# keyber/Single-Image-Super-Resolution

Measured on AMD Instinct MI355X. Metric: HR patches/sec (x2 generator fwd+bwd, LR 96x96 -> SR 192x192), higher is better.
Workload: dtype f32; 1 GPU; SRGAN x2 generator (16 blocks, 64 features, spectral norm) fwd+bwd+Adam with bicubic LR degradation and pixel-MSE x10, per-GPU batch 16 HR 192x192 patches (LR 96x96 -> SR 192x192): the north star's headline. BASELINE.json's metric string "96^2 crops, x4" is configs.cfg3 of this line. Single build: fp32.; per_gpu_batch=16, hr=192, lr=96, parallelism=dp1, hip_graph=True

## Files before the change

single-image-super-resolution_amd/csrc/conv_trunk_f32.hip:

```cpp
#include "sisr_dev.h"
#include "sisr_bf16_stage.h"
#include "sisr_instr.h"

typedef unsigned cf_u32x4 __attribute__((ext_vector_type(4)));

#include <algorithm>
#include <cstdlib>
#include <type_traits>

#define CF_TH 8
#define CF_TW 16
#define CF_IH (CF_TH + 2)
#define CF_IW (CF_TW + 2)
#define CF_NPIX (CF_IH * CF_IW)
#define CF_PSF 36
#define CF_HALO_BYTES (CF_NPIX * CF_PSF * 4)
#define CF_WROW 36
#define CF_WCHUNK_BYTES (9 * 32 * CF_WROW * 4)
#define CF_ITEMS ((CF_NPIX * 8 + 255) / 256)
#define CF_THREADS 512
#define CF_KROWP 100
#define CF_PS 33

SISR_TRACE_BUFFER(sisr_cftrace, 512, 128)
#define CFT(k) SISR_TRACE_STAMP(sisr_cftrace, threadIdx.x == 0, blockIdx.x, k, 64, wall_clock64())
#define CFTP(k) SISR_TRACE_STAMP(sisr_cftrace, threadIdx.x == 256, blockIdx.x, 64 + (k), 128, wall_clock64())
SISR_TRACE_BUFFER(sisr_cfclk, 512, 2)
#define CFTC(k) SISR_TRACE_STAMP(sisr_cfclk, threadIdx.x == 0, blockIdx.x, (k) - 60, 2, clock64())

struct CTrunkF32Args {
    const float *x1, *x2;
    float* x_out;
    BnFinArgs fin;
    const float *pa, *pb, *pd, *ps, *pt;
    const float* slope_p; float slope;
    const float* wpk;
    const void* wimg;
    const float* bias;
    const float* res;
    float* y;
    float *stat_part, *cnt_part;
    const float *bnb_x, *bnb_scale, *bnb_shift, *bnb_mean, *bnb_invstd, *bnb_slope_p;
    float bnb_slope; int bnb_act;
    float* bnb_part;
    int N, H, W;
    int tiles_x, per_img, total, streams;
    uint32_t m_tiles_x, m_per_img;
    int glog, cout_pad, shuffle;
    int xsc, xph;
};

__device__ __forceinline__ __amdgpu_buffer_rsrc_t cf_rsrc(const void* p, unsigned bytes) {
    return __builtin_amdgcn_make_buffer_rsrc(const_cast<void*>(p), 0, (int)bytes, 0x00020000);
}

__device__ __forceinline__ void cf_split2(float v0, float v1, unsigned& hw, unsigned& lw) {
    const f32x2 v = {v0, v1};
    hw = __builtin_bit_cast(unsigned, __builtin_convertvector(v, bf16x2));
    const f32x2 r = {v0 - __uint_as_float(hw << 16), v1 - __uint_as_float(hw & 0xFFFF0000u)};
    lw = __builtin_bit_cast(unsigned, __builtin_convertvector(r, bf16x2));
}

template <int PRO, bool SPLIT>
__global__ void __launch_bounds__(CF_THREADS, 2) conv_trunk_f32_kernel(const CTrunkF32Args a) {
    extern __shared__ __attribute__((aligned(16))) unsigned char lds[];
    unsigned char* halo0 = lds + 2 * CF_WCHUNK_BYTES;
    float* red = reinterpret_cast<float*>(halo0 + 2 * CF_HALO_BYTES);

    const int tid = threadIdx.x, lane = tid & 63;
    const int wave = __builtin_amdgcn_readfirstlane(tid >> 6);
    const bool consumer = wave < 4;
    const int l31 = lane & 31, kk = lane >> 5;
    const bool xcd = (a.streams & 7) == 0;
    const int hc = xcd ? (blockIdx.x >> 3) & ((1 << a.glog) - 1) : blockIdx.x & ((1 << a.glog) - 1);
    const int stream = xcd ? (blockIdx.x & 7) | ((blockIdx.x >> (3 + a.glog)) << 3) : blockIdx.x >> a.glog;
    const unsigned tbytes = (unsigned)a.N * (unsigned)a.H * (unsigned)a.W * 256u;
    constexpr bool TWO = PRO == SISR_PRO_BNBWD || PRO == SISR_PRO_BNACT_BWD || PRO == SISR_PRO_RES_AFFINE || PRO == SISR_PRO_ACT_BWD;
    constexpr bool SUM = PRO == SISR_PRO_RES_AFFINE;
    auto tile_coords = [&](int T, int& n, int& ty, int& tx) {
        n = fdiv(T, a.m_per_img);
        const int rem = T - n * a.per_img;
        ty = fdiv(rem, a.m_tiles_x);
        tx = rem - ty * a.tiles_x;
    };

    CFT(0);
    CFTC(60);
    float* kfin = red + 4 * 32 * 3;
    const bool fin = (PRO == SISR_PRO_AFFINE_ACT || PRO == SISR_PRO_RES_AFFINE) && a.fin.stat != nullptr;
    if (fin) bn_finalize_in_kernel(a.fin, reinterpret_cast<double*>(lds), kfin, blockIdx.x == 0);
    auto fill_weights = [&]() {
        float* wl = reinterpret_cast<float*>(lds);
        if (a.wimg != nullptr) {
            constexpr int UNITS = 2 * 9 * 32 * CF_WROW / 4;
            constexpr int W_IT16 = (UNITS + CF_THREADS - 1) / CF_THREADS;
            const cf_u32x4* src = reinterpret_cast<const cf_u32x4*>(a.wimg) + hc * UNITS;
            cf_u32x4 wv16[W_IT16];
#pragma unroll
            for (int it = 0; it < W_IT16; ++it) {
                const int u = tid + it * CF_THREADS;
                wv16[it] = u < UNITS ? src[u] : cf_u32x4{0u, 0u, 0u, 0u};
            }
#pragma unroll
            for (int it = 0; it < W_IT16; ++it) {
                const int u = tid + it * CF_THREADS;
                if (u < UNITS) reinterpret_cast<cf_u32x4*>(wl)[u] = wv16[it];
            }
            return;
        }
        constexpr int W_IT = 2 * 9 * 32 * 32 / CF_THREADS;
        float wv[W_IT];
#pragma unroll
        for (int it = 0; it < W_IT; ++it) {
            const int e = tid + it * CF_THREADS;
            const int ci = e & 31, s = (e >> 5) % 3, t2 = (e >> 5) / 3;
            const int co = t2 & 31, qr = t2 >> 5;
            wv[it] = a.wpk[((int64_t)qr * a.cout_pad + 32 * hc + co) * CF_KROWP + s * CF_PS + ci];
        }
#pragma unroll
        for (int it = 0; it < W_IT; ++it) {
            const int e = tid + it * CF_THREADS;
            const int ci = e & 31, s = (e >> 5) % 3, t2 = (e >> 5) / 3;
            const int co = t2 & 31, qr = t2 >> 5;
            const int q = qr / 3, r = qr - 3 * q;
            if constexpr (SPLIT) {
                const float vo = __shfl_xor(wv[it], 1);
                const bool odd = ci & 1;
                unsigned hw, lw;
                cf_split2(odd ? vo : wv[it], odd ? wv[it] : vo, hw, lw);
                reinterpret_cast<unsigned*>(wl)[((q * 9 + r * 3 + s) * 32 + co) * CF_WROW + (odd ? 16 : 0) + (ci >> 1)] = odd ? lw : hw;
            } else {
                wl[((q * 9 + r * 3 + s) * 32 + co) * CF_WROW + ci] = wv[it];
            }
        }
    };

    const int n_mine = stream < a.total ? (a.total - stream + a.streams - 1) / a.streams : 0;
    const int n_stages = 2 * n_mine;

    if (!consumer) {
        const int pt = tid & 255, quad = tid & 7, m0 = pt >> 3;
        const int tiles_y = a.per_img / a.tiles_x;
        const float slope = PRO != SISR_PRO_NONE ? (a.slope_p ? a.slope_p[0] : a.slope) : 1.f;
        f32x4 ka[2], kb[2], kd[2], ks[2], kt[2];
        int rel[CF_ITEMS];
        unsigned flags = 0;
#pragma unroll
        for (int k = 0; k < CF_ITEMS; ++k) {
            const int px = m0 + 32 * k;
            const int py = px / CF_IW, pxx = px - py * CF_IW;
            rel[k] = ((py - 1) * a.xsc * a.xsc * a.W + (pxx - 1) * a.xsc) * 256 + quad * 16;
            const unsigned f = (py == 0 ? 1u : 0u) | (py == CF_IH - 1 ? 2u : 0u) | (pxx == 0 ? 4u : 0u) | (pxx == CF_IW - 1 ? 8u : 0u) |
                               (px >= CF_NPIX ? 16u : 0u);
            flags |= f << (5 * k);
            asm volatile("" : "+v"(rel[k]));
        }
        const bool last_beyond = m0 + 32 * (CF_ITEMS - 1) >= CF_NPIX;
        const int ldso = SPLIT ? m0 * CF_PSF * 4 + quad * 8 : (m0 * CF_PSF + quad * 4) * 4;
        const bool easy_slope = slope >= 0.f && slope <= 1.f;

        struct Stage { f32x4 s1[CF_ITEMS], s2[CF_ITEMS]; unsigned bad, origin; bool edge; };
        Stage stA, stB;
        auto issue = [&](int j, Stage& st) {
            const int T = stream + (j >> 1) * a.streams, q = j & 1;
            const unsigned xbytes = (unsigned)(a.xsc * a.xsc) * tbytes;
            const __amdgpu_buffer_rsrc_t r1 = cf_rsrc(a.x1, xbytes), r2 = cf_rsrc(TWO ? a.x2 : a.x1, xbytes);
            int n, ty, tx;
            tile_coords(T, n, ty, tx);
            const unsigned origin = (unsigned)(((n * a.xsc * a.H + a.xsc * ty * CF_TH + (a.xph >> 1)) * a.xsc * a.W + a.xsc * tx * CF_TW + (a.xph & 1)) * 256 + q * 128);
            const unsigned e = (ty == 0 ? 1u : 0u) | (ty == tiles_y - 1 ? 2u : 0u) | (tx == 0 ? 4u : 0u) | (tx == a.tiles_x - 1 ? 8u : 0u);
            st.edge = e != 0u;
            st.bad = flags & ((e | 16u) * 0x02108421u);
            st.origin = origin;
#pragma unroll
            for (int k = 0; k < CF_ITEMS; ++k) {
                const unsigned voff = origin + (unsigned)rel[k];
                st.s1[k] = __builtin_bit_cast(f32x4, __builtin_amdgcn_raw_buffer_load_b128(r1, voff, 0, 0));
                if (TWO) st.s2[k] = __builtin_bit_cast(f32x4, __builtin_amdgcn_raw_buffer_load_b128(r2, voff, 0, 0));
            }
        };
        auto commit_t = [&](auto easy_, auto edge_, int j, const Stage& st) {
            constexpr int EASY = decltype(easy_)::value;
            constexpr bool EDGE = decltype(edge_)::value;
            const int q = j & 1;
            float* img = reinterpret_cast<float*>(halo0 + (j & 1) * CF_HALO_BYTES + ldso);
            const f32x4 qa = q ? ka[1] : ka[0], qb = q ? kb[1] : kb[0], qd = q ? kd[1] : kd[0], qs = q ? ks[1] : ks[0], qt = q ? kt[1] : kt[0];
            const __amdgpu_buffer_rsrc_t ro = cf_rsrc(SUM ? a.x_out : a.x1, tbytes);
#pragma unroll
            for (int k = 0; k < CF_ITEMS; ++k) {
                if (k == CF_ITEMS - 1 && last_beyond) break;
                const bool ok = !EDGE || ((st.bad >> (5 * k)) & 31u) == 0u;
                auto value = [&](int c) {
                    const float v = st.s1[k][c];
                    if (PRO == SISR_PRO_NONE) return v;
                    if (PRO == SISR_PRO_ACT) return lrelu_t<EASY>(v, slope);
                    if (PRO == SISR_PRO_AFFINE_ACT) return lrelu_t<EASY>(qa[c] * v + qd[c], slope);
                    if (SUM) return lrelu_t<EASY>(v, slope) + (qa[c] * st.s2[k][c] + qd[c]);
                    if (PRO == SISR_PRO_ACT_BWD) return st.s2[k][c] > 0.f ? v : slope * v;
                    const float bx = st.s2[k][c];
                    float g = v;
                    if (PRO == SISR_PRO_BNACT_BWD) g = qs[c] * bx + qt[c] > 0.f ? v : slope * v;
                    return qa[c] * g + qb[c] * bx + qd[c];
                };
                const f32x4 osum = {value(0), value(1), value(2), value(3)};
                const f32x4 zero4 = {0.f, 0.f, 0.f, 0.f};
                if constexpr (SPLIT) {
                    typedef unsigned cf_u32x2 __attribute__((ext_vector_type(2)));
                    unsigned h0, l0, h1, l1;
                    cf_split2(osum[0], osum[1], h0, l0);
                    cf_split2(osum[2], osum[3], h1, l1);
                    const cf_u32x2 hw = {h0, h1}, lw = {l0, l1};
                    const cf_u32x2 z2 = {0u, 0u};
                    *reinterpret_cast<cf_u32x2*>(img + k * 32 * CF_PSF) = ok ? hw : z2;
                    *reinterpret_cast<cf_u32x2*>(img + k * 32 * CF_PSF + 16) = ok ? lw : z2;
                } else
                *reinterpret_cast<f32x4*>(img + k * 32 * CF_PSF) = ok ? osum : zero4;
                if (SUM && hc == 0 && ((flags >> (5 * k)) & 31u) == 0u)
                    __builtin_amdgcn_raw_buffer_store_b128(__builtin_bit_cast(cf_u32x4, osum), ro, st.origin + (unsigned)rel[k], 0, 0);
            }
        };
        auto commit = [&](int j, const Stage& st) {
            using T1 = std::integral_constant<int, 1>; using T0 = std::integral_constant<int, 0>;
            constexpr bool HAS_ACT = PRO == SISR_PRO_ACT || PRO == SISR_PRO_AFFINE_ACT || SUM;
            if (!HAS_ACT || easy_slope) {
                if (st.edge) commit_t(T1{}, std::true_type{}, j, st); else commit_t(T1{}, std::false_type{}, j, st);
            } else {
                if (st.edge) commit_t(T0{}, std::true_type{}, j, st); else commit_t(T0{}, std::false_type{}, j, st);
            }
        };

        issue(0, stA);
        issue(1, stB);
#pragma unroll
        for (int q = 0; q < 2; ++q)
#pragma unroll
            for (int j = 0; j < 4; ++j) {
                const int c = q * 32 + quad * 4 + j;
                constexpr bool AFF = PRO == SISR_PRO_AFFINE_ACT || (TWO && PRO != SISR_PRO_ACT_BWD);
                ka[q][j] = fin ? kfin[c] : AFF ? a.pa[c] : 1.f;
                kd[q][j] = fin ? kfin[64 + c] : AFF ? a.pd[c] : 0.f;
                kb[q][j] = (TWO && !SUM && PRO != SISR_PRO_ACT_BWD) ? a.pb[c] : 0.f;
                ks[q][j] = PRO == SISR_PRO_BNACT_BWD ? a.ps[c] : 0.f;
                kt[q][j] = PRO == SISR_PRO_BNACT_BWD ? a.pt[c] : 0.f;
            }
        fill_weights();
        __syncthreads();
        if (n_stages > 0) commit(0, stA);
        __syncthreads();
        int j = 0;
        while (j < n_stages) {
            CFTP(4 + 6 * j);
            issue(j + 2, stA);
            CFTP(5 + 6 * j);
            if (j + 1 < n_stages) commit(j + 1, stB);
            CFTP(8 + 6 * j);
            __syncthreads();
            CFTP(9 + 6 * j);
            if (++j >= n_stages) break;
            CFTP(4 + 6 * j);
            issue(j + 2, stB);
            CFTP(5 + 6 * j);
            if (j + 1 < n_stages) commit(j + 1, stA);
            CFTP(8 + 6 * j);
            __syncthreads();
            CFTP(9 + 6 * j);
            ++j;
        }
    } else {
        const int co = a.shuffle ? 32 * (hc & 1) + l31 : 32 * hc + l31;
        const int ph = hc >> 1;
        const int abase = SPLIT ? ((2 * wave + (l31 >> 4)) * CF_IW + (l31 & 15)) * CF_PSF * 4 + 16 * kk
                                : (((2 * wave + (l31 >> 4)) * CF_IW + (l31 & 15)) * CF_PSF + 16 * kk) * 4;
        const int bbase = SPLIT ? l31 * CF_WROW * 4 + 16 * kk : (l31 * CF_WROW + 16 * kk) * 4;
        const float bv = a.bias != nullptr ? a.bias[a.shuffle ? co * 4 + ph : co] : 0.f;
        float st_shift = 0.f, st_s1 = 0.f, st_s2 = 0.f;
        int st_n = 0;
        const __amdgpu_buffer_rsrc_t ry = cf_rsrc(a.y, a.shuffle ? 4u * tbytes : tbytes), rr = cf_rsrc(a.res != nullptr ? a.res : a.y, tbytes);
        f32x16 acc;
        f32x16 rv, xv;
        const bool has_x = a.bnb_part != nullptr;
        const __amdgpu_buffer_rsrc_t rxb = cf_rsrc(has_x ? a.bnb_x : a.y, tbytes);
        float b_sc = 0.f, b_sf = 0.f, b_mu = 0.f, b_is = 0.f, b_slope = 1.f;
        float rs1 = 0.f, rs2 = 0.f, rsl = 0.f;
        if (has_x) {
            b_sc = a.bnb_scale[co]; b_sf = a.bnb_shift[co]; b_mu = a.bnb_mean[co]; b_is = a.bnb_invstd[co];
            b_slope = a.bnb_slope_p ? a.bnb_slope_p[0] : a.bnb_slope;
        }
        fill_weights();
        __syncthreads();
        __syncthreads();
        for (int j = 0; j < n_stages; ++j) {
            const int q = j & 1;
            CFT(4 + 6 * j);
            int n, ty, tx;
            tile_coords(stream + (j >> 1) * a.streams, n, ty, tx);
            const unsigned obase = a.shuffle ? (unsigned)((((n * 2 * a.H + 2 * (ty * CF_TH + 2 * wave) + (ph >> 1)) * 2 * a.W + 2 * tx * CF_TW + (ph & 1)) * 64 + co) * 4)
                                             : (unsigned)((((n * a.H + ty * CF_TH + 2 * wave) * a.W + tx * CF_TW) * 64 + co) * 4);
            const int orow = a.shuffle ? 4 * a.W * 256 : a.W * 256, ocol = a.shuffle ? 512 : 256;
            if (q == 0) {
#pragma unroll
                for (int i = 0; i < 16; ++i) acc[i] = bv;
            } else {
                if (a.res != nullptr) {
#pragma unroll
                    for (int i = 0; i < 16; ++i) {
                        const int p = mfma_row(i, lane);
                        rv[i] = __builtin_bit_cast(float, __builtin_amdgcn_raw_buffer_load_b32(rr, obase + (unsigned)(((p >> 4) * a.W + (p & 15)) * 256), 0, 0));
                    }
                }
                if (has_x) {
#pragma unroll
                    for (int i = 0; i < 16; ++i) {
                        const int p = mfma_row(i, lane);
                        xv[i] = __builtin_bit_cast(float, __builtin_amdgcn_raw_buffer_load_b32(rxb, obase + (unsigned)(((p >> 4) * a.W + (p & 15)) * 256), 0, 0));
                    }
                }
            }
            const unsigned char* ab = halo0 + (j & 1) * CF_HALO_BYTES + abase;
            const unsigned char* bb = lds + q * CF_WCHUNK_BYTES + bbase;
            if constexpr (SPLIT) {
                bf16x8 ah[9][2], al[9][2], bh[9][2], bl[9][2];
                auto fetch_s = [&](int t) {
                    const unsigned char* pa = ab + ((t / 3) * CF_IW + (t % 3)) * CF_PSF * 4;
                    const unsigned char* pb = bb + t * 32 * CF_WROW * 4;
#pragma unroll
                    for (int ks = 0; ks < 2; ++ks) {
                        ah[t][ks] = *reinterpret_cast<const bf16x8*>(pa + 32 * ks);
                        bh[t][ks] = *reinterpret_cast<const bf16x8*>(pb + 32 * ks);
                        al[t][ks] = *reinterpret_cast<const bf16x8*>(pa + 64 + 32 * ks);
                        bl[t][ks] = *reinterpret_cast<const bf16x8*>(pb + 64 + 32 * ks);
                    }
                };
                fetch_s(0);
                fetch_s(1);
                __builtin_amdgcn_sched_barrier(0);
#pragma unroll
                for (int t = 0; t < 9; ++t) {
                    if (t + 2 < 9) fetch_s(t + 2);
#pragma unroll
                    for (int ks = 0; ks < 2; ++ks) {
                        acc = __builtin_amdgcn_mfma_f32_32x32x16_bf16(al[t][ks], bh[t][ks], acc, 0, 0, 0);
                        acc = __builtin_amdgcn_mfma_f32_32x32x16_bf16(ah[t][ks], bl[t][ks], acc, 0, 0, 0);
                        acc = __builtin_amdgcn_mfma_f32_32x32x16_bf16(ah[t][ks], bh[t][ks], acc, 0, 0, 0);
                    }
                    __builtin_amdgcn_sched_barrier(0);
                }
            } else {
            f32x4 af[18][2], bf[18][2];
            auto fetch = [&](int u) {
                const int t = u >> 1, s0 = 8 * (u & 1);
#pragma unroll
                for (int v = 0; v < 2; ++v) {
                    af[u][v] = *reinterpret_cast<const f32x4*>(ab + (((t / 3) * CF_IW + (t % 3)) * CF_PSF + s0 + 4 * v) * 4);
                    bf[u][v] = *reinterpret_cast<const f32x4*>(bb + ((t * 32) * CF_WROW + s0 + 4 * v) * 4);
                }
            };
            fetch(0);
            fetch(1);
            __builtin_amdgcn_sched_group_barrier(0x100, 8, 0);
#pragma unroll
            for (int u = 0; u < 18; ++u) {
                if (u + 2 < 18) fetch(u + 2);
#pragma unroll
                for (int s = 0; s < 8; ++s) acc = __builtin_amdgcn_mfma_f32_32x32x2f32(af[u][s >> 2][s & 3], bf[u][s >> 2][s & 3], acc, 0, 0, 0);
                if (u + 2 < 18) __builtin_amdgcn_sched_group_barrier(0x100, 4, 0);
                __builtin_amdgcn_sched_group_barrier(0x008, 8, 0);
            }
            }
            CFT(6 + 6 * j);
            if (q == 1) {
                if (a.res != nullptr) {
#pragma unroll
                    for (int i = 0; i < 16; ++i) acc[i] += rv[i];
                }
                if (has_x) {
                    if (a.bnb_act) {
#pragma unroll
                        for (int i = 0; i < 16; ++i) {
                            float gv = acc[i];
                            const float z = b_sc * xv[i] + b_sf;
                            const bool neg = !(z > 0.f);
                            rsl += neg ? gv * z : 0.f;
                            gv = neg ? gv * b_slope : gv;
                            rs1 += gv;
                            rs2 += gv * ((xv[i] - b_mu) * b_is);
                        }
                    } else {
#pragma unroll
                        for (int i = 0; i < 16; ++i) {
                            rs1 += acc[i];
                            rs2 += acc[i] * ((xv[i] - b_mu) * b_is);
                        }
                    }
                }
                if (a.stat_part != nullptr) {
                    if (st_n == 0) {
                        float s = 0.f;
#pragma unroll
                        for (int i = 0; i < 16; ++i) s += acc[i];
                        st_shift = s * (1.f / 16.f);
                    }
#pragma unroll
                    for (int i = 0; i < 16; ++i) {
                        const float dv = acc[i] - st_shift;
                        st_s1 += dv;
                        st_s2 += dv * dv;
                    }
                    st_n += 16;
                }
#pragma unroll
                for (int i = 0; i < 16; ++i) {
                    const int p = mfma_row(i, lane);
                    __builtin_amdgcn_raw_buffer_store_b32(__builtin_bit_cast(unsigned, (float)acc[i]), ry,
                                                          obase + (unsigned)((p >> 4) * orow + (p & 15) * ocol), 0, 0);
                }
            }
            CFT(8 + 6 * j);
            __syncthreads();
            CFT(9 + 6 * j);
        }
        CFT(3);

        if (a.stat_part != nullptr) {
            float nn = (float)st_n, mu = 0.f, m2 = 0.f;
            if (st_n > 0) {
                const float m1 = st_s1 / nn;
                mu = st_shift + m1;
                m2 = st_s2 - st_s1 * m1;
            }
            const float nb = __shfl_xor(nn, 32), mub = __shfl_xor(mu, 32), m2b = __shfl_xor(m2, 32);
            const float nt = nn + nb;
            if (nt > 0.f) { const float dl = mub - mu, f = nb / nt; mu += dl * f; m2 += m2b + dl * dl * nn * f; }
            nn = nt;
            if (kk == 0) { float* r = red + (wave * 32 + l31) * 3; r[0] = nn; r[1] = mu; r[2] = m2; }
        }
        if (has_x) {
            rs1 += __shfl_xor(rs1, 32);
            rs2 += __shfl_xor(rs2, 32);
            rsl += __shfl_xor(rsl, 32);
            if (kk == 0) { float* r = red + (wave * 32 + l31) * 3; r[0] = rs1; r[1] = rs2; r[2] = rsl; }
        }
    }
    if (a.bnb_part != nullptr) {
        __syncthreads();
        float* wk = a.bnb_part + (int64_t)blockIdx.x * 129;
        if (tid < 64) {
            const int c = tid & 31;
            const bool mine = (tid >> 5) == hc;
            float s1 = 0.f, s2 = 0.f;
            if (mine) {
                s1 = (red[c * 3] + red[(32 + c) * 3]) + (red[(64 + c) * 3] + red[(96 + c) * 3]);
                s2 = (red[c * 3 + 1] + red[(32 + c) * 3 + 1]) + (red[(64 + c) * 3 + 1] + red[(96 + c) * 3 + 1]);
            }
            wk[tid] = s1;
            wk[64 + tid] = s2;
        }
        if (tid == 64) {
            float sl = 0.f;
            for (int i = 0; i < 128; ++i) sl += red[i * 3 + 2];
            wk[128] = sl;
        }
    }
    if (a.stat_part != nullptr) {
        __syncthreads();
        if (tid < 32) {
            float nn = red[tid * 3], mm = red[tid * 3 + 1], qq = red[tid * 3 + 2];
#pragma unroll
            for (int w = 1; w < 4; ++w) {
                const float* r1 = red + (w * 32 + tid) * 3;
                const float nb = r1[0], nt = nn + nb;
                if (nt > 0.f) { const float dl = r1[1] - mm, f = nb / nt; mm += dl * f; qq += r1[2] + dl * dl * nn * f; }
                nn = nt;
            }
            float* sp = a.stat_part + (int64_t)stream * 128 + 32 * hc + tid;
            sp[0] = mm;
            sp[64] = qq;
            if (tid == 0 && hc == 0) a.cnt_part[stream] = nn;
        }
    }
    CFT(63);
    CFTC(61);
}

static int cf_streams(const SisrConvDesc* d) {
    const int total = d->N * (d->H / CF_TH) * (d->W / CF_TW);
    const int cus = sisr_cu_slots();
    const int slots = std::max(1, cus / (d->Cout == 256 ? 8 : 2));
    const int rounds = (total + slots - 1) / slots;
    return (total + rounds - 1) / rounds;
}

extern "C" int sisr_conv2d_trunk_f32_eligible(const SisrConvDesc* d) {
    if (!d || sisr_switch_off("SISR_TRUNK")) return 0;
    if (sisr_switch_off("SISR_TRUNK_F32CONV")) return 0;
    const bool up_off = sisr_switch_off("SISR_TRUNK_UP");
    if (!up_off && d->Cin == 256 && d->Cout == 64 && d->KH == 3 && d->KW == 3 && d->stride == 1 && d->pad_y == 1 && d->pad_x == 1 &&
        d->x_mode == SISR_X_NHWC_UNSHUFFLE2 && d->pro_mode == SISR_PRO_ACT_BWD && d->x2 && d->y_mode == SISR_Y_NHWC && !d->x_bf16 && !d->y_bf16 &&
        !d->res_bf16 && d->Ho == d->H && d->Wo == d->W && !(d->H % CF_TH) && !(d->W % CF_TW) && d->y_sy == 1 && d->y_sx == 1 && !d->y_oy && !d->y_ox &&
        d->y_H == d->Ho && d->y_W == d->Wo && d->epi_act == SISR_EPI_NONE && d->plan.CK == 32 && d->plan.PS == CF_PS && d->plan.KROWP == CF_KROWP &&
        d->plan.CoutPad == 64 && d->plan.n_chunk == 8 && (int64_t)d->N * d->H * d->W * 1024 < (1ll << 31) &&
        d->N * (d->H / CF_TH) * (d->W / CF_TW) < 65536 && !d->stat_part && !d->bias && !d->bnb_part && !d->fin_stat)
        return 2;
    if (d->Cin != 64 || d->KH != 3 || d->KW != 3 || d->stride != 1 || d->pad_y != 1 || d->pad_x != 1) return 0;
    const bool up = !up_off && d->Cout == 256 && d->y_mode == SISR_Y_NHWC_SHUFFLE2 && d->plan.CoutPad == 256 && !d->stat_part &&
                    !d->res && !d->bnb_part && !d->fin_stat &&
                    (d->pro_mode == SISR_PRO_NONE || d->pro_mode == SISR_PRO_ACT || d->pro_mode == SISR_PRO_AFFINE_ACT);
    if (!up && (d->Cout != 64 || d->y_mode != SISR_Y_NHWC || d->plan.CoutPad != 64)) return 0;
    if (d->x_mode != SISR_X_NHWC || d->x_bf16 || d->y_bf16 || d->res_bf16) return 0;
    if (d->Ho != d->H || d->Wo != d->W || (d->H % CF_TH) || (d->W % CF_TW)) return 0;
    if (!up && (d->y_sy != 1 || d->y_sx != 1 || d->y_oy || d->y_ox || d->y_H != d->Ho || d->y_W != d->Wo)) return 0;
    if (d->epi_act != SISR_EPI_NONE) return 0;
    if (d->plan.CK != 32 || d->plan.PS != CF_PS || d->plan.KROWP != CF_KROWP || d->plan.n_chunk != 2) return 0;
    if ((int64_t)d->N * d->H * d->W * 256 * (up ? 4 : 1) >= (1ll << 31)) return 0;
    if (d->N * (d->H / CF_TH) * (d->W / CF_TW) >= 65536) return 0;
    const bool fwd_pro = d->pro_mode == SISR_PRO_NONE || d->pro_mode == SISR_PRO_ACT || d->pro_mode == SISR_PRO_AFFINE_ACT ||
                         (d->pro_mode == SISR_PRO_RES_AFFINE && d->x2 && d->x_out && ((d->pa && d->pd) || d->fin_stat));
    if (d->fin_stat && !((d->pro_mode == SISR_PRO_AFFINE_ACT || d->pro_mode == SISR_PRO_RES_AFFINE) && d->fin_cnt && d->fin_gamma &&
                         d->fin_beta && d->fin_rm && d->fin_rv && d->fin_k && d->fin_rows > 0))
        return 0;
    if (fwd_pro && !d->res && !d->bnb_part) return 1;
    const bool bwd_pro = d->pro_mode == SISR_PRO_BNBWD || d->pro_mode == SISR_PRO_BNACT_BWD;
    if (bwd_pro && !d->stat_part && !d->bias && (!d->bnb_part || (d->bnb_x && !d->bnbx_bf16))) return 2;
    return 0;
}

extern "C" int sisr_conv2d_f32_parts(const SisrConvDesc* d) {
    if (!d) return SISR_E_BADARG;
    return sisr_conv2d_trunk_f32_eligible(d) ? cf_streams(d) : d->plan.n_tiles;
}

extern "C" int sisr_conv2d_f32_bnb_parts(const SisrConvDesc* d) {
    if (!d) return SISR_E_BADARG;
    return sisr_conv2d_trunk_f32_eligible(d) == 2 ? 2 * cf_streams(d) : 0;
}

template <int PRO, bool SPLIT>
static int launch_cf_t(const CTrunkF32Args& a, hipStream_t st) {
    constexpr int lds_bytes = 2 * CF_WCHUNK_BYTES + 2 * CF_HALO_BYTES + 4 * 32 * 3 * 4 + 128 * 4;
    return sisr_launch<conv_trunk_f32_kernel<PRO, SPLIT>>(dim3(a.streams << a.glog), dim3(CF_THREADS), lds_bytes, 0, st, a);
}
template <int PRO>
static int launch_cf(const CTrunkF32Args& a, bool split, hipStream_t st) {
    return split ? launch_cf_t<PRO, true>(a, st) : launch_cf_t<PRO, false>(a, st);
}

int sisr_conv2d_trunk_f32_launch(const SisrConvDesc* d, hipStream_t st) {
    if (operand_needs_x2(d->pro_mode) && !d->x2) return SISR_E_BADARG;
    CTrunkF32Args a{};
    a.fin.stat = d->fin_stat; a.fin.cnt = d->fin_cnt; a.fin.gamma = d->fin_gamma; a.fin.beta = d->fin_beta;
    a.fin.rm = d->fin_rm; a.fin.rv = d->fin_rv; a.fin.k = d->fin_k; a.fin.rows = d->fin_rows; a.fin.momentum = d->fin_momentum; a.fin.eps = d->fin_eps;
    a.x1 = d->x1; a.x2 = d->x2; a.x_out = d->x_out; a.pa = d->pa; a.pb = d->pb; a.pd = d->pd; a.ps = d->ps; a.pt = d->pt;
    a.slope_p = d->pro_slope_p; a.slope = d->pro_slope;
    a.wpk = d->wpk; a.bias = d->bias; a.res = d->res; a.y = d->y; a.stat_part = d->stat_part; a.cnt_part = d->cnt_part;
    const int img_mode = (d->plan.variant >> 1) & 3;
    a.wimg = (d->Cin == 64 && d->Cout == 64 && img_mode == (d->mfma_split ? 2 : 1)) ? static_cast<const void*>(d->wpk + d->plan.wpk_elems) : nullptr;
    a.N = d->N; a.H = d->H; a.W = d->W;
    a.tiles_x = d->W / CF_TW; a.per_img = (d->H / CF_TH) * a.tiles_x; a.total = d->N * a.per_img;
    a.streams = cf_streams(d);
    a.glog = d->Cout == 256 ? 3 : 1; a.cout_pad = d->Cout == 256 ? 256 : 64; a.shuffle = d->y_mode == SISR_Y_NHWC_SHUFFLE2 ? 1 : 0;
    a.bnb_x = d->bnb_x; a.bnb_scale = d->bnb_scale; a.bnb_shift = d->bnb_shift; a.bnb_mean = d->bnb_mean; a.bnb_invstd = d->bnb_invstd;
    a.bnb_slope_p = d->bnb_slope_p; a.bnb_slope = d->bnb_slope; a.bnb_act = d->bnb_act; a.bnb_part = d->bnb_part;
    a.m_tiles_x = fdiv_magic(a.tiles_x); a.m_per_img = fdiv_magic(a.per_img);
    a.xsc = 1; a.xph = 0;
    if (d->Cin == 256) {
        a.xsc = 2;
        for (int ph = 0; ph < 4; ++ph) {
            a.xph = ph;
            a.wpk = d->wpk + (size_t)ph * 2 * 3 * 64 * CF_KROWP;
            a.res = ph == 0 ? d->res : d->y;
            if (int e = launch_cf<SISR_PRO_ACT_BWD>(a, d->mfma_split != 0, st)) return e;
        }
        return 0;
    }
    switch (d->pro_mode) {
        case SISR_PRO_NONE: return launch_cf<SISR_PRO_NONE>(a, d->mfma_split != 0, st);
        case SISR_PRO_ACT: return launch_cf<SISR_PRO_ACT>(a, d->mfma_split != 0, st);
        case SISR_PRO_AFFINE_ACT: return launch_cf<SISR_PRO_AFFINE_ACT>(a, d->mfma_split != 0, st);
        case SISR_PRO_BNBWD: return launch_cf<SISR_PRO_BNBWD>(a, d->mfma_split != 0, st);
        case SISR_PRO_BNACT_BWD: return launch_cf<SISR_PRO_BNACT_BWD>(a, d->mfma_split != 0, st);
        case SISR_PRO_RES_AFFINE: return launch_cf<SISR_PRO_RES_AFFINE>(a, d->mfma_split != 0, st);
    }
    return SISR_E_UNSUPPORTED;
}
```

Baseline: 1453 HR patches/s.

## Widen trunk conv tiles to 48 columns with swizzled 16-channel halo stages

Adds a template group count G so each tile covers 16*G columns (G=3 when W is a multiple of 48 and the wave-quantization check passes), giving each consumer wave G accumulators that reuse the same weight fragments. The halo is restaged in four 16-channel slices with an XOR-swizzled pixel layout instead of two 32-channel padded rows, and the per-channel affine constants move from producer registers into an LDS table. The intent is to amortize weight LDS reads and per-tile overhead over more output pixels and cut bank conflicts. The cost is more LDS per block, more registers per consumer, and fewer tiles, which can hurt load balance across CUs.

After: 1452 HR patches/s. Within noise of the previous version (-0.1%).

```diff
diff --git a/single-image-super-resolution_amd/csrc/conv_trunk_f32.hip b/single-image-super-resolution_amd/csrc/conv_trunk_f32.hip
--- a/single-image-super-resolution_amd/csrc/conv_trunk_f32.hip
+++ b/single-image-super-resolution_amd/csrc/conv_trunk_f32.hip
@@ -9,18 +9,31 @@
 #include <type_traits>
 
 #define CF_TH 8
-#define CF_TW 16
 #define CF_IH (CF_TH + 2)
-#define CF_IW (CF_TW + 2)
-#define CF_NPIX (CF_IH * CF_IW)
-#define CF_PSF 36
-#define CF_HALO_BYTES (CF_NPIX * CF_PSF * 4)
+#define CF_SC 16
+#define CF_NST (64 / CF_SC)
+#define CF_PIXB (CF_SC * 4)
 #define CF_WROW 36
 #define CF_WCHUNK_BYTES (9 * 32 * CF_WROW * 4)
-#define CF_ITEMS ((CF_NPIX * 8 + 255) / 256)
 #define CF_THREADS 512
 #define CF_KROWP 100
 #define CF_PS 33
+#define CF_RED_BYTES (4 * 32 * 3 * 4)
+#define CF_KTAB_BYTES (5 * 64 * 4)
+
+template <int G>
+struct CfGeom {
+    static constexpr int TW = 16 * G, IW = TW + 2, IWP = (IW + 3) & ~3, NPIX = CF_IH * IW;
+    static constexpr int ROWB = IWP * CF_PIXB;
+    static constexpr int HALO_BYTES = CF_IH * ROWB;
+    static constexpr int ITEMS = (NPIX * 4 + 255) / 256;
+    static constexpr int LDS_BYTES = 2 * CF_WCHUNK_BYTES + 2 * HALO_BYTES + CF_RED_BYTES + CF_KTAB_BYTES;
+    static_assert(LDS_BYTES <= 160 * 1024, "LDS budget");
+    static_assert(ITEMS * 4 <= 32, "four edge bits per item in one word");
+    static_assert((ITEMS - 2) * 64 + 63 < NPIX, "only a thread's last item may lie beyond the halo");
+    static_assert(HALO_BYTES + 2 * ROWB + 2 * 1024 + 64 < 65536, "operand fetch offsets fit the ds immediate");
+};
+__host__ __device__ __forceinline__ constexpr int cf_swz(int u) { return ((u >> 2) & 3) ^ (u & 2); }
 
 SISR_TRACE_BUFFER(sisr_cftrace, 512, 128)
 #define CFT(k) SISR_TRACE_STAMP(sisr_cftrace, threadIdx.x == 0, blockIdx.x, k, 64, wall_clock64())
@@ -61,11 +74,14 @@
     lw = __builtin_bit_cast(unsigned, __builtin_convertvector(r, bf16x2));
 }
 
-template <int PRO, bool SPLIT>
+template <int PRO, bool SPLIT, int G>
 __global__ void __launch_bounds__(CF_THREADS, 2) conv_trunk_f32_kernel(const CTrunkF32Args a) {
+    using Geo = CfGeom<G>;
+    constexpr int IW = Geo::IW, IWP = Geo::IWP, NPIX = Geo::NPIX, ROWB = Geo::ROWB, HALO_BYTES = Geo::HALO_BYTES, ITEMS = Geo::ITEMS;
     extern __shared__ __attribute__((aligned(16))) unsigned char lds[];
     unsigned char* halo0 = lds + 2 * CF_WCHUNK_BYTES;
-    float* red = reinterpret_cast<float*>(halo0 + 2 * CF_HALO_BYTES);
+    float* red = reinterpret_cast<float*>(halo0 + 2 * HALO_BYTES);
+    float* ktab = red + CF_RED_BYTES / 4;
 
     const int tid = threadIdx.x, lane = tid & 63;
     const int wave = __builtin_amdgcn_readfirstlane(tid >> 6);
@@ -77,6 +93,8 @@
     const unsigned tbytes = (unsigned)a.N * (unsigned)a.H * (unsigned)a.W * 256u;
     constexpr bool TWO = PRO == SISR_PRO_BNBWD || PRO == SISR_PRO_BNACT_BWD || PRO == SISR_PRO_RES_AFFINE || PRO == SISR_PRO_ACT_BWD;
     constexpr bool SUM = PRO == SISR_PRO_RES_AFFINE;
+    constexpr bool BWD = PRO == SISR_PRO_BNBWD || PRO == SISR_PRO_BNACT_BWD || PRO == SISR_PRO_ACT_BWD;
+    constexpr bool BNB = PRO == SISR_PRO_BNBWD || PRO == SISR_PRO_BNACT_BWD;
     auto tile_coords = [&](int T, int& n, int& ty, int& tx) {
         n = fdiv(T, a.m_per_img);
         const int rem = T - n * a.per_img;
@@ -86,9 +104,14 @@
 
     CFT(0);
     CFTC(60);
-    float* kfin = red + 4 * 32 * 3;
     const bool fin = (PRO == SISR_PRO_AFFINE_ACT || PRO == SISR_PRO_RES_AFFINE) && a.fin.stat != nullptr;
-    if (fin) bn_finalize_in_kernel(a.fin, reinterpret_cast<double*>(lds), kfin, blockIdx.x == 0);
+    if (fin) bn_finalize_in_kernel(a.fin, reinterpret_cast<double*>(lds), ktab, blockIdx.x == 0);
+    if (tid < 64) {
+        constexpr bool AFF = PRO == SISR_PRO_AFFINE_ACT || (TWO && PRO != SISR_PRO_ACT_BWD);
+        if (AFF && !fin) { ktab[tid] = a.pa[tid]; ktab[64 + tid] = a.pd[tid]; }
+        if (TWO && !SUM && PRO != SISR_PRO_ACT_BWD) ktab[128 + tid] = a.pb[tid];
+        if (PRO == SISR_PRO_BNACT_BWD) { ktab[192 + tid] = a.ps[tid]; ktab[256 + tid] = a.pt[tid]; }
+    }
     auto fill_weights = [&]() {
         float* wl = reinterpret_cast<float*>(lds);
         if (a.wimg != nullptr) {
@@ -136,44 +159,43 @@
     };
 
     const int n_mine = stream < a.total ? (a.total - stream + a.streams - 1) / a.streams : 0;
-    const int n_stages = 2 * n_mine;
+    const int n_stages = CF_NST * n_mine;
 
     if (!consumer) {
-        const int pt = tid & 255, quad = tid & 7, m0 = pt >> 3;
+        const int pt = tid & 255, quad = tid & 3, m0 = pt >> 2;
         const int tiles_y = a.per_img / a.tiles_x;
         const float slope = PRO != SISR_PRO_NONE ? (a.slope_p ? a.slope_p[0] : a.slope) : 1.f;
-        f32x4 ka[2], kb[2], kd[2], ks[2], kt[2];
-        int rel[CF_ITEMS];
+        int rel[ITEMS], ldso[ITEMS];
         unsigned flags = 0;
 #pragma unroll
-        for (int k = 0; k < CF_ITEMS; ++k) {
-            const int px = m0 + 32 * k;
-            const int py = px / CF_IW, pxx = px - py * CF_IW;
+        for (int k = 0; k < ITEMS; ++k) {
+            const int px = m0 + 64 * k;
+            const int py = px / IW, pxx = px - py * IW;
             rel[k] = ((py - 1) * a.xsc * a.xsc * a.W + (pxx - 1) * a.xsc) * 256 + quad * 16;
-            const unsigned f = (py == 0 ? 1u : 0u) | (py == CF_IH - 1 ? 2u : 0u) | (pxx == 0 ? 4u : 0u) | (pxx == CF_IW - 1 ? 8u : 0u) |
-                               (px >= CF_NPIX ? 16u : 0u);
-            flags |= f << (5 * k);
-            asm volatile("" : "+v"(rel[k]));
-        }
-        const bool last_beyond = m0 + 32 * (CF_ITEMS - 1) >= CF_NPIX;
-        const int ldso = SPLIT ? m0 * CF_PSF * 4 + quad * 8 : (m0 * CF_PSF + quad * 4) * 4;
+            ldso[k] = (py * IWP + pxx) * CF_PIXB + (SPLIT ? (((quad >> 1) ^ cf_swz(pxx)) << 4) + 8 * (quad & 1) : (quad ^ cf_swz(pxx)) << 4);
+            const unsigned f = (py == 0 ? 1u : 0u) | (py == CF_IH - 1 ? 2u : 0u) | (pxx == 0 ? 4u : 0u) | (pxx == IW - 1 ? 8u : 0u);
+            flags |= f << (4 * k);
+            asm volatile("" : "+v"(rel[k]), "+v"(ldso[k]));
+        }
+        const bool last_beyond = m0 + 64 * (ITEMS - 1) >= NPIX;
         const bool easy_slope = slope >= 0.f && slope <= 1.f;
-
-        struct Stage { f32x4 s1[CF_ITEMS], s2[CF_ITEMS]; unsigned bad, origin; bool edge; };
+        const float* kq = ktab + 4 * quad;
+
+        struct Stage { f32x4 s1[ITEMS], s2[ITEMS]; unsigned bad, origin; bool edge; };
         Stage stA, stB;
         auto issue = [&](int j, Stage& st) {
-            const int T = stream + (j >> 1) * a.streams, q = j & 1;
+            const int T = stream + (j >> 2) * a.streams, q = j & 3;
             const unsigned xbytes = (unsigned)(a.xsc * a.xsc) * tbytes;
             const __amdgpu_buffer_rsrc_t r1 = cf_rsrc(a.x1, xbytes), r2 = cf_rsrc(TWO ? a.x2 : a.x1, xbytes);
             int n, ty, tx;
             tile_coords(T, n, ty, tx);
-            const unsigned origin = (unsigned)(((n * a.xsc * a.H + a.xsc * ty * CF_TH + (a.xph >> 1)) * a.xsc * a.W + a.xsc * tx * CF_TW + (a.xph & 1)) * 256 + q * 128);
+            const unsigned origin = (unsigned)(((n * a.xsc * a.H + a.xsc * ty * CF_TH + (a.xph >> 1)) * a.xsc * a.W + a.xsc * tx * Geo::TW + (a.xph & 1)) * 256 + q * CF_PIXB);
             const unsigned e = (ty == 0 ? 1u : 0u) | (ty == tiles_y - 1 ? 2u : 0u) | (tx == 0 ? 4u : 0u) | (tx == a.tiles_x - 1 ? 8u : 0u);
             st.edge = e != 0u;
-            st.bad = flags & ((e | 16u) * 0x02108421u);
+            st.bad = flags & (e * 0x11111111u);
             st.origin = origin;
 #pragma unroll
-            for (int k = 0; k < CF_ITEMS; ++k) {
+            for (int k = 0; k < ITEMS; ++k) {
                 const unsigned voff = origin + (unsigned)rel[k];
                 st.s1[k] = __builtin_bit_cast(f32x4, __builtin_amdgcn_raw_buffer_load_b128(r1, voff, 0, 0));
                 if (TWO) st.s2[k] = __builtin_bit_cast(f32x4, __builtin_amdgcn_raw_buffer_load_b128(r2, voff, 0, 0));
@@ -182,14 +204,17 @@
         auto commit_t = [&](auto easy_, auto edge_, int j, const Stage& st) {
             constexpr int EASY = decltype(easy_)::value;
             constexpr bool EDGE = decltype(edge_)::value;
-            const int q = j & 1;
-            float* img = reinterpret_cast<float*>(halo0 + (j & 1) * CF_HALO_BYTES + ldso);
-            const f32x4 qa = q ? ka[1] : ka[0], qb = q ? kb[1] : kb[0], qd = q ? kd[1] : kd[0], qs = q ? ks[1] : ks[0], qt = q ? kt[1] : kt[0];
+            const int q = j & 3;
+            unsigned char* img = halo0 + (j & 1) * HALO_BYTES;
+            const float* kj = kq + CF_SC * q;
+            const f32x4 qa = *reinterpret_cast<const f32x4*>(kj), qd = *reinterpret_cast<const f32x4*>(kj + 64),
+                        qb = *reinterpret_cast<const f32x4*>(kj + 128), qs = *reinterpret_cast<const f32x4*>(kj + 192),
+                        qt = *reinterpret_cast<const f32x4*>(kj + 256);
             const __amdgpu_buffer_rsrc_t ro = cf_rsrc(SUM ? a.x_out : a.x1, tbytes);
 #pragma unroll
-            for (int k = 0; k < CF_ITEMS; ++k) {
-                if (k == CF_ITEMS - 1 && last_beyond) break;
-                const bool ok = !EDGE || ((st.bad >> (5 * k)) & 31u) == 0u;
+            for (int k = 0; k < ITEMS; ++k) {
+                if (k == ITEMS - 1 && last_beyond) break;
+                const bool ok = !EDGE || ((st.bad >> (4 * k)) & 15u) == 0u;
                 auto value = [&](int c) {
                     const float v = st.s1[k][c];
                     if (PRO == SISR_PRO_NONE) return v;
@@ -211,11 +236,11 @@
                     cf_split2(osum[2], osum[3], h1, l1);
                     const cf_u32x2 hw = {h0, h1}, lw = {l0, l1};
                     const cf_u32x2 z2 = {0u, 0u};
-                    *reinterpret_cast<cf_u32x2*>(img + k * 32 * CF_PSF) = ok ? hw : z2;
-                    *reinterpret_cast<cf_u32x2*>(img + k * 32 * CF_PSF + 16) = ok ? lw : z2;
+                    *reinterpret_cast<cf_u32x2*>(img + ldso[k]) = ok ? hw : z2;
+                    *reinterpret_cast<cf_u32x2*>(img + (ldso[k] ^ 32)) = ok ? lw : z2;
                 } else
-                *reinterpret_cast<f32x4*>(img + k * 32 * CF_PSF) = ok ? osum : zero4;
-                if (SUM && hc == 0 && ((flags >> (5 * k)) & 31u) == 0u)
+                *reinterpret_cast<f32x4*>(img + ldso[k]) = ok ? osum : zero4;
+                if (SUM && hc == 0 && ((flags >> (4 * k)) & 15u) == 0u)
                     __builtin_amdgcn_raw_buffer_store_b128(__builtin_bit_cast(cf_u32x4, osum), ro, st.origin + (unsigned)rel[k], 0, 0);
             }
         };
@@ -229,21 +254,11 @@
             }
         };
 
+        constexpr bool LATE1 = TWO && G > 1;
         issue(0, stA);
-        issue(1, stB);
-#pragma unroll
-        for (int q = 0; q < 2; ++q)
-#pragma unroll
-            for (int j = 0; j < 4; ++j) {
-                const int c = q * 32 + quad * 4 + j;
-                constexpr bool AFF = PRO == SISR_PRO_AFFINE_ACT || (TWO && PRO != SISR_PRO_ACT_BWD);
-                ka[q][j] = fin ? kfin[c] : AFF ? a.pa[c] : 1.f;
-                kd[q][j] = fin ? kfin[64 + c] : AFF ? a.pd[c] : 0.f;
-                kb[q][j] = (TWO && !SUM && PRO != SISR_PRO_ACT_BWD) ? a.pb[c] : 0.f;
-                ks[q][j] = PRO == SISR_PRO_BNACT_BWD ? a.ps[c] : 0.f;
-                kt[q][j] = PRO == SISR_PRO_BNACT_BWD ? a.pt[c] : 0.f;
-            }
+        if (!LATE1) issue(1, stB);
         fill_weights();
+        if (LATE1) issue(1, stB);
         __syncthreads();
         if (n_stages > 0) commit(0, stA);
         __syncthreads();
@@ -269,16 +284,24 @@
     } else {
         const int co = a.shuffle ? 32 * (hc & 1) + l31 : 32 * hc + l31;
         const int ph = hc >> 1;
-        const int abase = SPLIT ? ((2 * wave + (l31 >> 4)) * CF_IW + (l31 & 15)) * CF_PSF * 4 + 16 * kk
-                                : (((2 * wave + (l31 >> 4)) * CF_IW + (l31 & 15)) * CF_PSF + 16 * kk) * 4;
-        const int bbase = SPLIT ? l31 * CF_WROW * 4 + 16 * kk : (l31 * CF_WROW + 16 * kk) * 4;
-        const float bv = a.bias != nullptr ? a.bias[a.shuffle ? co * 4 + ph : co] : 0.f;
+        int ao[3][2];
+#pragma unroll
+        for (int tc = 0; tc < 3; ++tc)
+#pragma unroll
+            for (int v = 0; v < 2; ++v) {
+                const int u = (l31 & 15) + tc, slot = SPLIT ? 2 * v + kk : 2 * kk + v;
+                ao[tc][v] = ((2 * wave + (l31 >> 4)) * IWP + u) * CF_PIXB + ((slot ^ cf_swz(u)) << 4);
+                asm volatile("" : "+v"(ao[tc][v]));
+            }
+        const unsigned char* bbase = lds + l31 * CF_WROW * 4 + (SPLIT ? 16 * kk : 32 * kk);
+        const float bv = !BWD && a.bias != nullptr ? a.bias[a.shuffle ? co * 4 + ph : co] : 0.f;
         float st_shift = 0.f, st_s1 = 0.f, st_s2 = 0.f;
         int st_n = 0;
         const __amdgpu_buffer_rsrc_t ry = cf_rsrc(a.y, a.shuffle ? 4u * tbytes : tbytes), rr = cf_rsrc(a.res != nullptr ? a.res : a.y, tbytes);
-        f32x16 acc;
-        f32x16 rv, xv;
-        const bool has_x = a.bnb_part != nullptr;
+        f32x16 acc[G];
+        const bool has_res = BWD && a.res != nullptr;
+        const bool has_x = BNB && a.bnb_part != nullptr;
+        const bool has_stat = !BWD && a.stat_part != nullptr;
         const __amdgpu_buffer_rsrc_t rxb = cf_rsrc(has_x ? a.bnb_x : a.y, tbytes);
         float b_sc = 0.f, b_sf = 0.f, b_mu = 0.f, b_is = 0.f, b_slope = 1.f;
         float rs1 = 0.f, rs2 = 0.f, rsl = 0.f;
@@ -286,123 +309,62 @@
             b_sc = a.bnb_scale[co]; b_sf = a.bnb_shift[co]; b_mu = a.bnb_mean[co]; b_is = a.bnb_invstd[co];
             b_slope = a.bnb_slope_p ? a.bnb_slope_p[0] : a.bnb_slope;
         }
-        fill_weights();
-        __syncthreads();
-        __syncthreads();
-        for (int j = 0; j < n_stages; ++j) {
-            const int q = j & 1;
-            CFT(4 + 6 * j);
-            int n, ty, tx;
-            tile_coords(stream + (j >> 1) * a.streams, n, ty, tx);
-            const unsigned obase = a.shuffle ? (unsigned)((((n * 2 * a.H + 2 * (ty * CF_TH + 2 * wave) + (ph >> 1)) * 2 * a.W + 2 * tx * CF_TW + (ph & 1)) * 64 + co) * 4)
-                                             : (unsigned)((((n * a.H + ty * CF_TH + 2 * wave) * a.W + tx * CF_TW) * 64 + co) * 4);
-            const int orow = a.shuffle ? 4 * a.W * 256 : a.W * 256, ocol = a.shuffle ? 512 : 256;
-            if (q == 0) {
-#pragma unroll
-                for (int i = 0; i < 16; ++i) acc[i] = bv;
-            } else {
-                if (a.res != nullptr) {
+        unsigned obase_kk = 0;
+        const int orow = a.shuffle ? 4 * a.W * 256 : a.W * 256, ocol = a.shuffle ? 512 : 256;
+        auto stage = [&](auto buf_, int j) __attribute__((always_inline)) {
+            constexpr int BUF = decltype(buf_)::value;
+            const int h = j & 3;
+            f32x16 rv[G], xv[G];
+            auto request = [&](int g) __attribute__((always_inline)) {
+                if (has_res) {
 #pragma unroll
                     for (int i = 0; i < 16; ++i) {
-                        const int p = mfma_row(i, lane);
-                        rv[i] = __builtin_bit_cast(float, __builtin_amdgcn_raw_buffer_load_b32(rr, obase + (unsigned)(((p >> 4) * a.W + (p & 15)) * 256), 0, 0));
+                        rv[g][i] = __builtin_bit_cast(float, __builtin_amdgcn_raw_buffer_load_b32(rr, obase_kk, ((i >> 3) * a.W + 16 * g + (i & 3) + 8 * ((i >> 2) & 1)) * 256, 0));
                     }
                 }
                 if (has_x) {
 #pragma unroll
                     for (int i = 0; i < 16; ++i) {
-                        const int p = mfma_row(i, lane);
-                        xv[i] = __builtin_bit_cast(float, __builtin_amdgcn_raw_buffer_load_b32(rxb, obase + (unsigned)(((p >> 4) * a.W + (p & 15)) * 256), 0, 0));
+                        xv[g][i] = __builtin_bit_cast(float, __builtin_amdgcn_raw_buffer_load_b32(rxb, obase_kk, ((i >> 3) * a.W + 16 * g + (i & 3) + 8 * ((i >> 2) & 1)) * 256, 0));
                     }
                 }
-            }
-            const unsigned char* ab = halo0 + (j & 1) * CF_HALO_BYTES + abase;
-            const unsigned char* bb = lds + q * CF_WCHUNK_BYTES + bbase;
-            if constexpr (SPLIT) {
-                bf16x8 ah[9][2], al[9][2], bh[9][2], bl[9][2];
-                auto fetch_s = [&](int t) {
-                    const unsigned char* pa = ab + ((t / 3) * CF_IW + (t % 3)) * CF_PSF * 4;
-                    const unsigned char* pb = bb + t * 32 * CF_WROW * 4;
-#pragma unroll
-                    for (int ks = 0; ks < 2; ++ks) {
-                        ah[t][ks] = *reinterpret_cast<const bf16x8*>(pa + 32 * ks);
-                        bh[t][ks] = *reinterpret_cast<const bf16x8*>(pb + 32 * ks);
-                        al[t][ks] = *reinterpret_cast<const bf16x8*>(pa + 64 + 32 * ks);
-                        bl[t][ks] = *reinterpret_cast<const bf16x8*>(pb + 64 + 32 * ks);
-                    }
-                };
-                fetch_s(0);
-                fetch_s(1);
-                __builtin_amdgcn_sched_barrier(0);
-#pragma unroll
-                for (int t = 0; t < 9; ++t) {
-                    if (t + 2 < 9) fetch_s(t + 2);
-#pragma unroll
-                    for (int ks = 0; ks < 2; ++ks) {
-                        acc = __builtin_amdgcn_mfma_f32_32x32x16_bf16(al[t][ks], bh[t][ks], acc, 0, 0, 0);
-                        acc = __builtin_amdgcn_mfma_f32_32x32x16_bf16(ah[t][ks], bl[t][ks], acc, 0, 0, 0);
-                        acc = __builtin_amdgcn_mfma_f32_32x32x16_bf16(ah[t][ks], bh[t][ks], acc, 0, 0, 0);
-                    }
-                    __builtin_amdgcn_sched_barrier(0);
-                }
-            } else {
-            f32x4 af[18][2], bf[18][2];
-            auto fetch = [&](int u) {
-                const int t = u >> 1, s0 = 8 * (u & 1);
-#pragma unroll
-                for (int v = 0; v < 2; ++v) {
-                    af[u][v] = *reinterpret_cast<const f32x4*>(ab + (((t / 3) * CF_IW + (t % 3)) * CF_PSF + s0 + 4 * v) * 4);
-                    bf[u][v] = *reinterpret_cast<const f32x4*>(bb + ((t * 32) * CF_WROW + s0 + 4 * v) * 4);
-                }
             };
-            fetch(0);
-            fetch(1);
-            __builtin_amdgcn_sched_group_barrier(0x100, 8, 0);
-#pragma unroll
-            for (int u = 0; u < 18; ++u) {
-                if (u + 2 < 18) fetch(u + 2);
-#pragma unroll
-                for (int s = 0; s < 8; ++s) acc = __builtin_amdgcn_mfma_f32_32x32x2f32(af[u][s >> 2][s & 3], bf[u][s >> 2][s & 3], acc, 0, 0, 0);
-                if (u + 2 < 18) __builtin_amdgcn_sched_group_barrier(0x100, 4, 0);
-                __builtin_amdgcn_sched_group_barrier(0x008, 8, 0);
-            }
-            }
-            CFT(6 + 6 * j);
-            if (q == 1) {
-                if (a.res != nullptr) {
-#pragma unroll
-                    for (int i = 0; i < 16; ++i) acc[i] += rv[i];
+            auto finish = [&](int g) __attribute__((always_inline)) {
+                f32x16& ac = acc[g];
+                if (has_res) {
+#pragma unroll
+                    for (int i = 0; i < 16; ++i) ac[i] += rv[g][i];
                 }
                 if (has_x) {
                     if (a.bnb_act) {
 #pragma unroll
                         for (int i = 0; i < 16; ++i) {
-                            float gv = acc[i];
-                            const float z = b_sc * xv[i] + b_sf;
+                            float gv = ac[i];
+                            const float z = b_sc * xv[g][i] + b_sf;
                             const bool neg = !(z > 0.f);
                             rsl += neg ? gv * z : 0.f;
                             gv = neg ? gv * b_slope : gv;
                             rs1 += gv;
-                            rs2 += gv * ((xv[i] - b_mu) * b_is);
+                            rs2 += gv * ((xv[g][i] - b_mu) * b_is);
                         }
                     } else {
 #pragma unroll
                         for (int i = 0; i < 16; ++i) {
-                            rs1 += acc[i];
-                            rs2 += acc[i] * ((xv[i] - b_mu) * b_is);
+                            rs1 += ac[i];
+                            rs2 += ac[i] * ((xv[g][i] - b_mu) * b_is);
                         }
                     }
                 }
-                if (a.stat_part != nullptr) {
+                if (has_stat) {
                     if (st_n == 0) {
                         float s = 0.f;
 #pragma unroll
-                        for (int i = 0; i < 16; ++i) s += acc[i];
+                        for (int i = 0; i < 16; ++i) s += ac[i];
                         st_shift = s * (1.f / 16.f);
                     }
 #pragma unroll
                     for (int i = 0; i < 16; ++i) {
-                        const float dv = acc[i] - st_shift;
+                        const float dv = ac[i] - st_shift;
                         st_s1 += dv;
                         st_s2 += dv * dv;
                     }
@@ -410,18 +372,113 @@
                 }
 #pragma unroll
                 for (int i = 0; i < 16; ++i) {
-                    const int p = mfma_row(i, lane);
-                    __builtin_amdgcn_raw_buffer_store_b32(__builtin_bit_cast(unsigned, (float)acc[i]), ry,
-                                                          obase + (unsigned)((p >> 4) * orow + (p & 15) * ocol), 0, 0);
+                    __builtin_amdgcn_raw_buffer_store_b32(__builtin_bit_cast(unsigned, (float)ac[i]), ry, obase_kk,
+                                                          (i >> 3) * orow + (16 * g + (i & 3) + 8 * ((i >> 2) & 1)) * ocol, 0);
+                }
+            };
+            CFT(4 + 6 * j);
+            if (h == 0) {
+                int n, ty, tx;
+                tile_coords(stream + (j >> 2) * a.streams, n, ty, tx);
+                const unsigned obase = a.shuffle ? (unsigned)((((n * 2 * a.H + 2 * (ty * CF_TH + 2 * wave) + (ph >> 1)) * 2 * a.W + 2 * tx * Geo::TW + (ph & 1)) * 64 + co) * 4)
+                                             : (unsigned)((((n * a.H + ty * CF_TH + 2 * wave) * a.W + tx * Geo::TW) * 64 + co) * 4);
+                obase_kk = obase + (unsigned)(4 * kk * ocol);
+#pragma unroll
+                for (int g = 0; g < G; ++g)
+#pragma unroll
+                    for (int i = 0; i < 16; ++i) acc[g][i] = bv;
+            }
+            const unsigned char* bb = bbase + (h >> 1) * CF_WCHUNK_BYTES + (h & 1) * (SPLIT ? 32 : 64);
+            auto a_at = [&](int t, int g, int v) { return halo0 + ao[t % 3][v] + BUF * HALO_BYTES + (t / 3) * ROWB + g * 16 * CF_PIXB; };
+            auto chains = [&](auto g0_, auto ng_) __attribute__((always_inline)) {
+                constexpr int G0 = decltype(g0_)::value, NG = decltype(ng_)::value;
+                if constexpr (SPLIT) {
+                    bf16x8 ah[9][NG], al[9][NG], bh[9], bl[9];
+                    auto fetch_s = [&](int t) {
+                        bh[t] = *reinterpret_cast<const bf16x8*>(bb + t * 32 * CF_WROW * 4);
+                        bl[t] = *reinterpret_cast<const bf16x8*>(bb + t * 32 * CF_WROW * 4 + 64);
+#pragma unroll
+                        for (int g = 0; g < NG; ++g) {
+                            ah[t][g] = *reinterpret_cast<const bf16x8*>(a_at(t, G0 + g, 0));
+                            al[t][g] = *reinterpret_cast<const bf16x8*>(a_at(t, G0 + g, 1));
+                        }
+                    };
+                    fetch_s(0);
+                    fetch_s(1);
+                    __builtin_amdgcn_sched_barrier(0);
+#pragma unroll
+                    for (int t = 0; t < 9; ++t) {
+                        if (t + 2 < 9) fetch_s(t + 2);
+#pragma unroll
+                        for (int g = 0; g < NG; ++g) acc[G0 + g] = __builtin_amdgcn_mfma_f32_32x32x16_bf16(al[t][g], bh[t], acc[G0 + g], 0, 0, 0);
+#pragma unroll
+                        for (int g = 0; g < NG; ++g) acc[G0 + g] = __builtin_amdgcn_mfma_f32_32x32x16_bf16(ah[t][g], bl[t], acc[G0 + g], 0, 0, 0);
+#pragma unroll
+                        for (int g = 0; g < NG; ++g) acc[G0 + g] = __builtin_amdgcn_mfma_f32_32x32x16_bf16(ah[t][g], bh[t], acc[G0 + g], 0, 0, 0);
+                        __builtin_amdgcn_sched_barrier(0);
+                    }
+                } else {
+                    f32x4 af[9][NG][2], bf[9][2];
+                    auto fetch = [&](int t) {
+#pragma unroll
+                        for (int v = 0; v < 2; ++v) bf[t][v] = *reinterpret_cast<const f32x4*>(bb + t * 32 * CF_WROW * 4 + 16 * v);
+#pragma unroll
+                        for (int g = 0; g < NG; ++g)
+#pragma unroll
+                            for (int v = 0; v < 2; ++v) af[t][g][v] = *reinterpret_cast<const f32x4*>(a_at(t, G0 + g, v));
+                    };
+                    fetch(0);
+                    __builtin_amdgcn_sched_group_barrier(0x100, 2 + 2 * NG, 0);
+#pragma unroll
+                    for (int t = 0; t < 9; ++t) {
+                        if (t + 1 < 9) fetch(t + 1);
+#pragma unroll
+                        for (int s = 0; s < 8; ++s)
+#pragma unroll
+                            for (int g = 0; g < NG; ++g)
+                                acc[G0 + g] = __builtin_amdgcn_mfma_f32_32x32x2f32(af[t][g][s >> 2][s & 3], bf[t][s >> 2][s & 3], acc[G0 + g], 0, 0, 0);
+                        if (t + 1 < 9) __builtin_amdgcn_sched_group_barrier(0x100, 2 + 2 * NG, 0);
+                        __builtin_amdgcn_sched_group_barrier(0x008, 8 * NG, 0);
+                    }
+                }
+            };
+            using I1 = std::integral_constant<int, 1>;
+            if (h != CF_NST - 1) {
+                chains(std::integral_constant<int, 0>{}, std::integral_constant<int, G>{});
+                CFT(6 + 6 * j);
+            } else {
+                if (BWD) request(0);
+                if (BWD && G > 1) request(1);
+                chains(std::integral_constant<int, 0>{}, I1{});
+                if constexpr (G > 1) {
+                    if (BWD && G > 2) request(2);
+                    finish(0);
+                    chains(I1{}, I1{});
+                    finish(1);
+                }
+                if constexpr (G > 2) {
+                    chains(std::integral_constant<int, 2>{}, I1{});
+                    CFT(6 + 6 * j);
+                    finish(2);
+                } else {
+                    CFT(6 + 6 * j);
+                    finish(G - 1);
                 }
             }
             CFT(8 + 6 * j);
             __syncthreads();
             CFT(9 + 6 * j);
+        };
+        fill_weights();
+        __syncthreads();
+        __syncthreads();
+        for (int j = 0; j < n_stages; j += 2) {
+            stage(std::integral_constant<int, 0>{}, j);
+            stage(std::integral_constant<int, 1>{}, j + 1);
         }
         CFT(3);
 
-        if (a.stat_part != nullptr) {
+        if (has_stat) {
             float nn = (float)st_n, mu = 0.f, m2 = 0.f;
             if (st_n > 0) {
                 const float m1 = st_s1 / nn;
@@ -441,7 +498,7 @@
             if (kk == 0) { float* r = red + (wave * 32 + l31) * 3; r[0] = rs1; r[1] = rs2; r[2] = rsl; }
         }
     }
-    if (a.bnb_part != nullptr) {
+    if (BNB && a.bnb_part != nullptr) {
         __syncthreads();
         float* wk = a.bnb_part + (int64_t)blockIdx.x * 129;
         if (tid < 64) {
@@ -461,7 +518,7 @@
             wk[128] = sl;
         }
     }
-    if (a.stat_part != nullptr) {
+    if (!BWD && a.stat_part != nullptr) {
         __syncthreads();
         if (tid < 32) {
             float nn = red[tid * 3], mm = red[tid * 3 + 1], qq = red[tid * 3 + 2];
@@ -482,10 +539,19 @@
     CFTC(61);
 }
 
+static int cf_slots(const SisrConvDesc* d) {
+    return std::max(1, sisr_cu_slots() / (d->Cout == 256 ? 8 : 2));
+}
+static int cf_groups(const SisrConvDesc* d) {
+    if (d->W % 48 || sisr_switch_off("SISR_TRUNK_F32_WIDE")) return 1;
+    const int slots = cf_slots(d);
+    const int total1 = d->N * (d->H / CF_TH) * (d->W / 16), total3 = total1 / 3;
+    const int rounds1 = (total1 + slots - 1) / slots, rounds3 = (total3 + slots - 1) / slots;
+    return 3 * rounds3 <= std::max(rounds1, 3) ? 3 : 1;
+}
 static int cf_streams(const SisrConvDesc* d) {
-    const int total = d->N * (d->H / CF_TH) * (d->W / CF_TW);
-    const int cus = sisr_cu_slots();
-    const int slots = std::max(1, cus / (d->Cout == 256 ? 8 : 2));
+    const int total = d->N * (d->H / CF_TH) * (d->W / (16 * cf_groups(d)));
+    const int slots = cf_slots(d);
     const int rounds = (total + slots - 1) / slots;
     return (total + rounds - 1) / rounds;
 }
@@ -496,10 +562,10 @@
     const bool up_off = sisr_switch_off("SISR_TRUNK_UP");
     if (!up_off && d->Cin == 256 && d->Cout == 64 && d->KH == 3 && d->KW == 3 && d->stride == 1 && d->pad_y == 1 && d->pad_x == 1 &&
         d->x_mode == SISR_X_NHWC_UNSHUFFLE2 && d->pro_mode == SISR_PRO_ACT_BWD && d->x2 && d->y_mode == SISR_Y_NHWC && !d->x_bf16 && !d->y_bf16 &&
-        !d->res_bf16 && d->Ho == d->H && d->Wo == d->W && !(d->H % CF_TH) && !(d->W % CF_TW) && d->y_sy == 1 && d->y_sx == 1 && !d->y_oy && !d->y_ox &&
+        !d->res_bf16 && d->Ho == d->H && d->Wo == d->W && !(d->H % CF_TH) && !(d->W % 16) && d->y_sy == 1 && d->y_sx == 1 && !d->y_oy && !d->y_ox &&
         d->y_H == d->Ho && d->y_W == d->Wo && d->epi_act == SISR_EPI_NONE && d->plan.CK == 32 && d->plan.PS == CF_PS && d->plan.KROWP == CF_KROWP &&
         d->plan.CoutPad == 64 && d->plan.n_chunk == 8 && (int64_t)d->N * d->H * d->W * 1024 < (1ll << 31) &&
-        d->N * (d->H / CF_TH) * (d->W / CF_TW) < 65536 && !d->stat_part && !d->bias && !d->bnb_part && !d->fin_stat)
+        d->N * (d->H / CF_TH) * (d->W / 16) < 65536 && !d->stat_part && !d->bias && !d->bnb_part && !d->fin_stat)
         return 2;
     if (d->Cin != 64 || d->KH != 3 || d->KW != 3 || d->stride != 1 || d->pad_y != 1 || d->pad_x != 1) return 0;
     const bool up = !up_off && d->Cout == 256 && d->y_mode == SISR_Y_NHWC_SHUFFLE2 && d->plan.CoutPad == 256 && !d->stat_part &&
@@ -507,12 +573,12 @@
                     (d->pro_mode == SISR_PRO_NONE || d->pro_mode == SISR_PRO_ACT || d->pro_mode == SISR_PRO_AFFINE_ACT);
     if (!up && (d->Cout != 64 || d->y_mode != SISR_Y_NHWC || d->plan.CoutPad != 64)) return 0;
     if (d->x_mode != SISR_X_NHWC || d->x_bf16 || d->y_bf16 || d->res_bf16) return 0;
-    if (d->Ho != d->H || d->Wo != d->W || (d->H % CF_TH) || (d->W % CF_TW)) return 0;
+    if (d->Ho != d->H || d->Wo != d->W || (d->H % CF_TH) || (d->W % 16)) return 0;
     if (!up && (d->y_sy != 1 || d->y_sx != 1 || d->y_oy || d->y_ox || d->y_H != d->Ho || d->y_W != d->Wo)) return 0;
     if (d->epi_act != SISR_EPI_NONE) return 0;
     if (d->plan.CK != 32 || d->plan.PS != CF_PS || d->plan.KROWP != CF_KROWP || d->plan.n_chunk != 2) return 0;
     if ((int64_t)d->N * d->H * d->W * 256 * (up ? 4 : 1) >= (1ll << 31)) return 0;
-    if (d->N * (d->H / CF_TH) * (d->W / CF_TW) >= 65536) return 0;
+    if (d->N * (d->H / CF_TH) * (d->W / 16) >= 65536) return 0;
     const bool fwd_pro = d->pro_mode == SISR_PRO_NONE || d->pro_mode == SISR_PRO_ACT || d->pro_mode == SISR_PRO_AFFINE_ACT ||
                          (d->pro_mode == SISR_PRO_RES_AFFINE && d->x2 && d->x_out && ((d->pa && d->pd) || d->fin_stat));
     if (d->fin_stat && !((d->pro_mode == SISR_PRO_AFFINE_ACT || d->pro_mode == SISR_PRO_RES_AFFINE) && d->fin_cnt && d->fin_gamma &&
@@ -534,14 +600,14 @@
     return sisr_conv2d_trunk_f32_eligible(d) == 2 ? 2 * cf_streams(d) : 0;
 }
 
-template <int PRO, bool SPLIT>
+template <int PRO, bool SPLIT, int G>
 static int launch_cf_t(const CTrunkF32Args& a, hipStream_t st) {
-    constexpr int lds_bytes = 2 * CF_WCHUNK_BYTES + 2 * CF_HALO_BYTES + 4 * 32 * 3 * 4 + 128 * 4;
-    return sisr_launch<conv_trunk_f32_kernel<PRO, SPLIT>>(dim3(a.streams << a.glog), dim3(CF_THREADS), lds_bytes, 0, st, a);
+    return sisr_launch<conv_trunk_f32_kernel<PRO, SPLIT, G>>(dim3(a.streams << a.glog), dim3(CF_THREADS), CfGeom<G>::LDS_BYTES, 0, st, a);
 }
 template <int PRO>
-static int launch_cf(const CTrunkF32Args& a, bool split, hipStream_t st) {
-    return split ? launch_cf_t<PRO, true>(a, st) : launch_cf_t<PRO, false>(a, st);
+static int launch_cf(const CTrunkF32Args& a, bool split, int groups, hipStream_t st) {
+    if (groups == 3) return split ? launch_cf_t<PRO, true, 3>(a, st) : launch_cf_t<PRO, false, 3>(a, st);
+    return split ? launch_cf_t<PRO, true, 1>(a, st) : launch_cf_t<PRO, false, 1>(a, st);
 }
 
 int sisr_conv2d_trunk_f32_launch(const SisrConvDesc* d, hipStream_t st) {
@@ -555,7 +621,8 @@
     const int img_mode = (d->plan.variant >> 1) & 3;
     a.wimg = (d->Cin == 64 && d->Cout == 64 && img_mode == (d->mfma_split ? 2 : 1)) ? static_cast<const void*>(d->wpk + d->plan.wpk_elems) : nullptr;
     a.N = d->N; a.H = d->H; a.W = d->W;
-    a.tiles_x = d->W / CF_TW; a.per_img = (d->H / CF_TH) * a.tiles_x; a.total = d->N * a.per_img;
+    const int groups = cf_groups(d);
+    a.tiles_x = d->W / (16 * groups); a.per_img = (d->H / CF_TH) * a.tiles_x; a.total = d->N * a.per_img;
     a.streams = cf_streams(d);
     a.glog = d->Cout == 256 ? 3 : 1; a.cout_pad = d->Cout == 256 ? 256 : 64; a.shuffle = d->y_mode == SISR_Y_NHWC_SHUFFLE2 ? 1 : 0;
     a.bnb_x = d->bnb_x; a.bnb_scale = d->bnb_scale; a.bnb_shift = d->bnb_shift; a.bnb_mean = d->bnb_mean; a.bnb_invstd = d->bnb_invstd;
@@ -568,17 +635,17 @@
             a.xph = ph;
             a.wpk = d->wpk + (size_t)ph * 2 * 3 * 64 * CF_KROWP;
             a.res = ph == 0 ? d->res : d->y;
-            if (int e = launch_cf<SISR_PRO_ACT_BWD>(a, d->mfma_split != 0, st)) return e;
+            if (int e = launch_cf<SISR_PRO_ACT_BWD>(a, d->mfma_split != 0, groups, st)) return e;
         }
         return 0;
     }
     switch (d->pro_mode) {
-        case SISR_PRO_NONE: return launch_cf<SISR_PRO_NONE>(a, d->mfma_split != 0, st);
-        case SISR_PRO_ACT: return launch_cf<SISR_PRO_ACT>(a, d->mfma_split != 0, st);
-        case SISR_PRO_AFFINE_ACT: return launch_cf<SISR_PRO_AFFINE_ACT>(a, d->mfma_split != 0, st);
-        case SISR_PRO_BNBWD: return launch_cf<SISR_PRO_BNBWD>(a, d->mfma_split != 0, st);
-        case SISR_PRO_BNACT_BWD: return launch_cf<SISR_PRO_BNACT_BWD>(a, d->mfma_split != 0, st);
-        case SISR_PRO_RES_AFFINE: return launch_cf<SISR_PRO_RES_AFFINE>(a, d->mfma_split != 0, st);
+        case SISR_PRO_NONE: return launch_cf<SISR_PRO_NONE>(a, d->mfma_split != 0, groups, st);
+        case SISR_PRO_ACT: return launch_cf<SISR_PRO_ACT>(a, d->mfma_split != 0, groups, st);
+        case SISR_PRO_AFFINE_ACT: return launch_cf<SISR_PRO_AFFINE_ACT>(a, d->mfma_split != 0, groups, st);
+        case SISR_PRO_BNBWD: return launch_cf<SISR_PRO_BNBWD>(a, d->mfma_split != 0, groups, st);
+        case SISR_PRO_BNACT_BWD: return launch_cf<SISR_PRO_BNACT_BWD>(a, d->mfma_split != 0, groups, st);
+        case SISR_PRO_RES_AFFINE: return launch_cf<SISR_PRO_RES_AFFINE>(a, d->mfma_split != 0, groups, st);
     }
     return SISR_E_UNSUPPORTED;
 }
```
